# Isomorpfishm/SINGA

Measured on AMD Instinct MI355X. Metric: protein-ligand graphs/sec GAN step (G+D fwd+bwd); scatter-TP kernel HBM GB/s, higher is better.
Workload: dtype f32

## Files before the change

### __graft_entry__.py

```python
import os
import subprocess
import sys

ROOT = os.path.dirname(os.path.abspath(__file__))
if ROOT not in sys.path:
    sys.path.insert(0, ROOT)

SRC = os.path.join(ROOT, "singa_amd", "csrc", "singa_hip.hip")
LIB = os.path.join(ROOT, "singa_amd", "lib", "libsinga_hip.so")


def build() -> None:
    os.makedirs(os.path.dirname(LIB), exist_ok=True)
    deps = [SRC, os.path.join(ROOT, "singa_amd", "csrc", "so3_index.h"), os.path.join(ROOT, "include", "singa_hip.h"),
            os.path.join(ROOT, "include", "singa_hip_lab.h"), os.path.join(ROOT, "include", "singa_hip_gen.h"),
            os.path.join(ROOT, "include", "singa_hip_force.h")]
    if not os.path.exists(LIB) or any(os.path.getmtime(d) > os.path.getmtime(LIB) for d in deps):
        hipcc = os.environ.get("HIPCC", "/opt/rocm/bin/hipcc")
        cmd = [hipcc, "--offload-arch=gfx950", "-O3", "-std=c++17", "-shared", "-fPIC", "-o", LIB, SRC]
        subprocess.check_call(cmd)
    import torch
    import singa_amd
    from singa_amd import _capi
    _capi.bind(LIB)


def smoke() -> None:
    import numpy as np
    import torch

    build()
    from oracle import singa_oracle as O
    from singa_amd import graph as G
    from singa_amd.config import load_config
    from singa_amd.model.GAN import SINGA
    from tests.helpers import golden, state_from_spec

    assert torch.cuda.is_available(), "smoke() needs a GPU"
    L = 2
    dev = "cuda:0"
    sd = state_from_spec(f"singa_L{L}")
    z = golden(f"singa_L{L}_B3.npz")
    names = ["3wi2_4tpp", "4agq_5a7b", "5cp5_4nue"]
    batch = G.collate([G.load_npz(os.path.join(ROOT, "tests", "golden", f"graph_{n}.npz"), with_lap=False) for n in names])
    batch.nodes[G.PA]["lap_pe"], batch.nodes[G.LA]["lap_pe"] = torch.tensor(z["lap_p"]), torch.tensor(z["lap_l"])
    batch.extras["edge_rot_mat"] = {k: torch.tensor(z[f"rot_{k}"]) for k in ("pp", "ll", "lp")}
    batch.extras["knn"] = {G.PA: torch.tensor(z["knn_p"]), G.LA: torch.tensor(z["knn_l"])}
    batch = batch.to(dev)
    model = SINGA(load_config(lmax=L), device=dev)
    model.load_state_dict(sd, strict=False)
    model.eval()
    logits = model(batch)
    loss = torch.nn.functional.cross_entropy(logits, batch["ligand_data"]["smiIndices_tgt"].reshape(-1))
    loss.backward()
    torch.cuda.synchronize()
    og = O.collate([O.load_graph_npz(os.path.join(ROOT, "tests", "golden", f"graph_{n}.npz")) for n in names])
    rots = {k: torch.as_tensor(z[f"rot_{k}"]) for k in ("pp", "ll", "lp")}
    with torch.no_grad():
        ref = O.singa_forward(sd, og, rots, L, torch.as_tensor(z["knn_p"]), torch.as_tensor(z["knn_l"]),
                              torch.as_tensor(z["lap_p"]), torch.as_tensor(z["lap_l"]))
    err = float((logits.detach().cpu().double() - ref.double()).norm() / ref.double().norm())
    gn = float(torch.sqrt(sum((p.grad.double() ** 2).sum() for p in model.parameters() if p.grad is not None)))
    print(f"smoke: loss {float(loss):.6f} (reference {float(z['loss']):.6f}), logits rel err vs oracle {err:.2e}, "
          f"grad norm {gn:.4f} (reference {float(z['grad_total']):.4f})")
    assert err < 1e-4, err
    assert abs(gn - float(z["grad_total"])) < 1e-4 * float(z["grad_total"])


if __name__ == "__main__":
    build()
    if len(sys.argv) > 1 and sys.argv[1] == "smoke":
        smoke()
```

### singa_amd/_capi.py

```python
import ctypes as C

P = C.c_void_p
I32 = C.c_int
I64 = C.c_int64
F32 = C.c_float


class Seg(C.Structure):
    _fields_ = [("ptr", P), ("ld", I64), ("rows", C.c_int32)]


SegArr = Seg * 3


class Gemm(C.Structure):
    _fields_ = [("a", P), ("b", P), ("c", P), ("bias", P), ("lda", I64), ("ldb", I64), ("ldc", I64), ("I", C.c_int32),
                ("J", C.c_int32), ("R", C.c_int32), ("a_group", C.c_int32), ("b_group", C.c_int32), ("c_group", C.c_int32),
                ("a_group_ld", I64), ("b_group_ld", I64), ("c_group_ld", I64), ("c_split_stride", I64), ("mask", P),
                ("addend", P), ("relu", C.c_int32), ("asum", P), ("asum_stride", I64)]


class CGemm(C.Structure):
    _fields_ = [("a", P), ("b", P), ("c", P), ("lda", I64), ("ldb", I64), ("ldc", I64), ("a_im", I64), ("b_im", I64),
                ("c_im", I64), ("c_split_stride", I64), ("I", C.c_int32), ("J", C.c_int32), ("R", C.c_int32),
# ... 33 lines not shown
    "singa_s2act_sep_fwd": ([C.POINTER(Seg), I32, P, I64, P, P, P, P, I32, I32, I32, P], I32),
    "singa_s2act_sep_bwd": ([C.POINTER(Seg), I32, P, I64, P, P, P, P, P, P, I32, I32, I32, P], I32),
    "singa_s2act_ffn_bwd": ([P, P, I64, P, P, P, P, P, P, I32, I32, I32, P], I32),
    "singa_s2act_sep_bwd_seg": ([C.POINTER(Seg), I32, P, I64, P, P, P, P, C.POINTER(Seg), P, I64, I32, I32, I32, P], I32),
    "singa_so3_rmsnorm_nparts": ([I32], I32),
    "singa_so3_rmsnorm_fwd": ([P, P, P, P, I32, I32, I32, F32, P], I32),
    "singa_so3_rmsnorm_bwd": ([P, P, P, P, P, P, I32, I32, I32, F32, P], I32),
    "singa_so3_rmsnorm_bwd_add": ([P, P, P, P, P, P, P, I32, I32, I32, F32, P], I32),
    "singa_edge_logits_fwd": ([P] * 7 + [I32, I32, I32, F32, P], I32),
    "singa_edge_logits_bwd": ([P] * 13 + [I32, I32, I32, F32, P], I32),
    "singa_gather_wsum_fwd": ([P] * 6 + [I32, I32, I32, P], I32),
    "singa_gather_wsum_bwd": ([P] * 12 + [I32, I32, I32, P], I32),
    "singa_bias_ssp_fwd": ([P] * 3 + [I64, I32, P], I32),
    "singa_bias_ssp_bwd": ([P] * 4 + [I64, I32, P], I32),
    "singa_dec_self_attn": ([P] * 10 + [I32, I32, P, F32, P], I32),
    "singa_dec_cross_attn": ([P] * 10 + [I32, I32, I32, P, F32, P], I32),
    "singa_dec_ffn": ([P] * 7 + [I32, P, F32, P], I32),
    "singa_sample_token": ([P, P, P, P, I32, I32, I32, I32, F32, I32, F32, I32, I32] + [P] * 8, I32),
    "singa_edge_mlp_fwd": ([P] * 11 + [I32, I32, I32, I32, P], I32),
    "singa_edge_mlp_bwd_nparts": ([I32, I32], I32),
    "singa_edge_mlp_bwd": ([P] * 6 + [I32, I32, I32, P], I32),
    "singa_masked_softmax_fwd": ([P, P, I64, I64, P, I32, I32, I32, I32, F32, P], I32),
    "singa_masked_softmax_bwd": ([P, P, P, I64, I64, P, I32, I32, I32, I32, F32, P], I32),
    "singa_attn_fwd": ([P, P, P, P, I64, I64, P, P, I32, I32, I32, I32, I32, I32, I32, I64, I64, I64, F32, P], I32),
    "singa_attn_bwd": ([P, P, P, P, I64, I64] + [P] * 7 + [I32, I32, I32, I32, I32, I32, I32, I64, I64, I64, F32, P], I32),
    "singa_ln256_nparts": ([I64], I32),
    "singa_ln256_fwd": ([P] * 5 + [I64, I32, F32, P], I32),
    "singa_ln256_bwd": ([P] * 6 + [I64, I32, F32, P], I32),
    "singa_ln_silu_nparts": ([I64], I32),
    "singa_ln_silu_fwd": ([P] * 4 + [I64, I32, F32, P], I32),
    "singa_ln_silu_bwd": ([P] * 6 + [I64, I32, F32, P], I32),
    "singa_colsum_work": ([C.c_longlong, I32], C.c_longlong),
    "singa_colsum": ([P, C.c_longlong, C.c_longlong, I32, P, P, P], I32),
    "singa_so3_skinny_nparts": ([I32, I32, I32], I32),
    "singa_so3_skinny_expand": ([P, P, I64, I64, I64, P, P, I32, I32, I32, P], I32),
    "singa_so3_skinny_reduce": ([P, P, P, I32, I32, I32, I32, I32, P], I32),
    "singa_colsum_multi_work": ([C.c_longlong, I32], C.c_longlong),
    "singa_colsum_multi": ([I32, P, P, P, P, P, I32, P, P, P, C.c_longlong, P], I32),
    "singa_block_weight_fwd": ([P, P, I32, I32, P], I32),
    "singa_block_weight_bwd": ([P, P, I32, I32, I32, P], I32),
    "singa_rowdot_nparts": ([C.c_longlong], I32),
    "singa_rowdot_fwd": ([P, P, P, C.c_longlong, I32, F32, P], I32),
    "singa_rowdot_bwd": ([P, P, P, P, P, C.c_longlong, I32, F32, P], I32),
    "singa_lap_pe_work": ([I32, I32], I32),
    "singa_lap_pe": ([P] * 8 + [I32, I32, I32, P], I32),
    "singa_adam_step": ([P, P, P, P, P, P, P, I32, I32, P, P, F32, F32, F32, P], I32),
    "singa_grad_norm": ([P, P, P, P, I32, I32, P, P, P], I32),
    "singa_gemm_f32": ([C.POINTER(Gemm), I32, I32, I32, I32, P], I32),
    "singa_cgemm3m_f32": ([C.POINTER(CGemm), I32, I32, I32, I32, P], I32),
    "singa_knn_graph": ([P, P, P, I32, I32, I32, I32, P, P, P], I32),
    "singa_knn_edge_attr": ([P, P, C.c_longlong, P, C.c_float, P, I32, I32, P], I32),
    "singa_prof_enable": ([I32], I32),
    "singa_prof_hint_edges": ([I32], I32),
    "singa_prof_collect": ([P, P, P, I32], I32),
    "singa_prof_collect_tagged": ([P, P, P, P, I32], I32),
    "singa_prof_stamps": ([P, I32], I32),
    "singa_prof_read_stamps": ([P, P, P, P, P, I32], I32),
    "singa_prof_reset": ([], I32),
    "singa_calib_copy": ([P, P, C.c_longlong, P], I32),
    "singa_calib_copy16": ([P, P, C.c_longlong, I32, I32, P], I32),
}

EXPORTS = tuple(_SIGS)

_LAB_SIGS = {
    "singa_so3_skinny_variant": ([I32], I32),
    "singa_gemm_occupancy": ([I32, I32, I32], I32),
    "singa_gemm_force_cfg": ([I32], I32),
    "singa_lap_pe_fsi_min": ([I32], I32),
}
LAB_EXPORTS = tuple(_LAB_SIGS)

_GEN_SIGS = {
    "singa_sample_token_grammar": ([P, P, P, P, P, I32, I32, I32, I32, F32, I32, F32, I32, I32] + [P] * 10, I32),
    "singa_smiles_rule_host": ([P, P, P, I32, P, P], I32),
}
GEN_EXPORTS = tuple(_GEN_SIGS)

_FORCE_SIGS = {
    "singa_sample_token_forced": ([P, P, P, P, P, I32, I32, I32, I32, F32, I32, F32, I32, I32] + [P] * 12, I32),
}
FORCE_EXPORTS = tuple(_FORCE_SIGS)


def bind(path):
    import torch
    lib = C.CDLL(path)
    for name, (args, res) in list(_SIGS.items()) + list(_LAB_SIGS.items()) + list(_GEN_SIGS.items()) + \
            list(_FORCE_SIGS.items()):
        fn = getattr(lib, name)
        fn.argtypes = args
        fn.restype = res
    return lib


def segs(items):
    arr = SegArr()
    for i, (p, ld, rows) in enumerate(items):
        arr[i].ptr, arr[i].ld, arr[i].rows = p, ld, rows
    return arr, len(items)


def check(lib, code, what):
    if code != 0:
        raise RuntimeError(f"{what} failed ({code}): {lib.singa_last_error_string().decode()}")
```

### singa_amd/csrc/singa_hip.hip

```cpp
#include <hip/hip_runtime.h>
#include <hip/hip_ext.h>

#include <math.h>
#include <stdint.h>
#include <stdio.h>
#include <string.h>
#include <type_traits>

#include "../../include/singa_hip.h"
#include "../../include/singa_hip_lab.h"
#include "../../include/singa_hip_gen.h"
#include "../../include/singa_hip_force.h"
#include "so3_index.h"

namespace {

thread_local char g_err[256] = "ok";

int fail(int code, const char* msg) {
    snprintf(g_err, sizeof(g_err), "%s", msg);
    return code;
}

int check_launch(const char* what) {
    hipError_t e = hipGetLastError();
    if (e != hipSuccess) {
        snprintf(g_err, sizeof(g_err), "%s: %s", what, hipGetErrorString(e));
        return (int)e;
    }
    return SINGA_OK;
}

struct ProfRec {
    hipEvent_t a, b;
    int E, N, tag;
};
constexpr int PROF_CAP = 8192;
ProfRec g_prof[PROF_CAP];
int g_prof_n = 0;
bool g_prof_on = false;
unsigned long long* g_stamp_buf = nullptr;
int g_stamp_cap = 0;
__global__ void stamp_kernel(unsigned long long* dst) { *dst = (unsigned long long)wall_clock64(); }
int g_prof_edges_hint = 0;

#ifndef SINGA_KEEP_VGPR
#define SINGA_KEEP_VGPR(x) __asm__ volatile("" : "+v"(x))
#endif

#define SINGA_LAUNCH(tag_, E_, N_, kern, grid, block, st, ...)                                                   \
    do {                                                                                                          \
        if (g_prof_on && g_prof_n < PROF_CAP) {                                                                   \
            ProfRec& r_ = g_prof[g_prof_n++];                                                                     \
            (void)hipEventCreate(&r_.a);                                                                          \
            (void)hipEventCreate(&r_.b);                                                                          \
            r_.E = (E_);                                                                                          \
            r_.N = (N_);                                                                                          \
            r_.tag = (tag_);                                                                                      \
            hipExtLaunchKernelGGL(kern, grid, block, 0, (st), r_.a, r_.b, 0, __VA_ARGS__);                        \
        } else if (g_stamp_buf && 2 * (g_prof_n + 2) <= g_stamp_cap && g_prof_n + 1 < PROF_CAP) {                 \
            if (g_prof_n == 0) {                                                                                  \
                g_prof[0].a = g_prof[0].b = nullptr;                                                              \
                g_prof[0].E = g_prof[0].N = g_prof[0].tag = 0;                                                    \
                hipLaunchKernelGGL(stamp_kernel, dim3(1), dim3(1), 0, (st), g_stamp_buf);                         \
                hipLaunchKernelGGL(stamp_kernel, dim3(1), dim3(1), 0, (st), g_stamp_buf + 1);                     \
                g_prof_n = 1;                                                                                     \
            }                                                                                                     \
            ProfRec& r_ = g_prof[g_prof_n];                                                                       \
            r_.a = r_.b = nullptr;                                                                                \
            r_.E = (E_);                                                                                          \
            r_.N = (N_);                                                                                          \
            r_.tag = (tag_);                                                                                      \
            hipLaunchKernelGGL(stamp_kernel, dim3(1), dim3(1), 0, (st), g_stamp_buf + 2 * g_prof_n);              \
            hipLaunchKernelGGL(kern, grid, block, 0, (st), __VA_ARGS__);                                          \
            hipLaunchKernelGGL(stamp_kernel, dim3(1), dim3(1), 0, (st), g_stamp_buf + 2 * g_prof_n + 1);          \
            ++g_prof_n;                                                                                           \
        } else                                                                                                    \
            hipLaunchKernelGGL(kern, grid, block, 0, (st), __VA_ARGS__);                                          \
    } while (0)

__device__ __forceinline__ int xcd_range_id(int vb, int n8) { return (vb & 7) * (n8 >> 3) + (vb >> 3); }
constexpr int MAX_J = 2300;
__device__ float g_J[MAX_J];
int g_lmax_init = -1;

__host__ __device__ constexpr int j_off(int l) {
    int s = 0;
    for (int i = 0; i < l; ++i) s += (2 * i + 1) * (2 * i + 1);
    return s;
}

struct Segs {
    const float* p[3];
    long long ld[3];
    int rows[3];
// ... 3207 lines not shown
        auto load = [&](float4* b, float* a, int q, int ch) {
            const int n = q + g;
            const bool ok = n < n1;
            const long long nn = ok ? n : n1 - 1;
#pragma unroll
            for (int d = 0; d < D; ++d) {
                const int k = ch * D + d;
                b[d] = *reinterpret_cast<const float4*>(big + (nn * K + k) * C + cc);
                const float v = small[(nn * K + k) * 16 + i];
                a[d] = ok ? v : 0.f;
            }
        };
        load(bnxt, anxt, n0, 0);
        for (int q = n0; q < n1; q += 4) {
#pragma unroll
            for (int ch = 0; ch < NCH; ++ch) {
#pragma unroll
                for (int d = 0; d < D; ++d) bcur[d] = bnxt[d], acur[d] = anxt[d];
                if (ch + 1 < NCH) load(bnxt, anxt, q, ch + 1);
                else load(bnxt, anxt, q + 4 < n1 ? q + 4 : q, 0);
#pragma unroll
                for (int d = 0; d < D; ++d) {
                    const int k = ch * D + d;
                    int l = 0;
                    while ((l + 1) * (l + 1) <= k) ++l;
                    const float bv[4] = {bcur[d].x, bcur[d].y, bcur[d].z, bcur[d].w};
#pragma unroll
                    for (int t = 0; t < 4; ++t) acc[l][t] = __builtin_amdgcn_mfma_f32_16x16x4f32(acur[d], bv[t], acc[l][t], 0, 0, 0);
                    if (k == 0 && q + g < n1) {
                        accb.x += bv[0]; accb.y += bv[1]; accb.z += bv[2]; accb.w += bv[3];
                    }
                }
            }
        }
    }
    constexpr int WSZ_ = (L + 1) * 16 * C;
    float* p = part + (long long)(blockIdx.x / HV) * (WSZ_ + (bias_row ? C : 0));
    if (bias_row) {
        accb.x += __shfl_xor(accb.x, 16, 64); accb.y += __shfl_xor(accb.y, 16, 64); accb.z += __shfl_xor(accb.z, 16, 64); accb.w += __shfl_xor(accb.w, 16, 64);
        accb.x += __shfl_xor(accb.x, 32, 64); accb.y += __shfl_xor(accb.y, 32, 64); accb.z += __shfl_xor(accb.z, 32, 64); accb.w += __shfl_xor(accb.w, 32, 64);
    }
    if (!act) return;
#pragma unroll
    for (int l = 0; l <= L; ++l) {
        if (out_cu) {
#pragma unroll
            for (int t = 0; t < 4; ++t)
                *reinterpret_cast<float4*>(p + ((long long)l * C + cc + t) * 16 + 4 * g) = make_float4(acc[l][t][0], acc[l][t][1], acc[l][t][2], acc[l][t][3]);
        } else {
#pragma unroll
            for (int r = 0; r < 4; ++r)
                *reinterpret_cast<float4*>(p + ((long long)l * 16 + 4 * g + r) * C + cc) = make_float4(acc[l][0][r], acc[l][1][r], acc[l][2][r], acc[l][3][r]);
        }
    }
    if (bias_row && g == 0) *reinterpret_cast<float4*>(p + WSZ_ + cc) = accb;
}

static inline int so3_skinny_npb(int N, int target_blocks) {
    int npb = (N + target_blocks - 1) / target_blocks;
    return npb < 8 ? 8 : npb;
}

template <int C>
static int so3_skinny_reduce_runs(int lmax) {
    static int cached[8] = {0};
    if (lmax < 0 || lmax > 7) return 512;
    if (cached[lmax]) return cached[lmax];
    int per_cu = 0, cus = 256;
    hipError_t e = hipErrorInvalidValue;
    constexpr int BL = SkinnyCfg<C>::BLOCK;
    if (lmax == 2) e = hipOccupancyMaxActiveBlocksPerMultiprocessor(&per_cu, so3_skinny_reduce_kernel<2, C>, BL, 0);
    if (lmax == 4) e = hipOccupancyMaxActiveBlocksPerMultiprocessor(&per_cu, so3_skinny_reduce_kernel<4, C>, BL, 0);
    if (lmax == 6) e = hipOccupancyMaxActiveBlocksPerMultiprocessor(&per_cu, so3_skinny_reduce_kernel<6, C>, BL, 0);
    if (e != hipSuccess || per_cu < 1) per_cu = 2;
    int dev = 0;
    hipDeviceProp_t prop;
    if (hipGetDevice(&dev) == hipSuccess && hipGetDeviceProperties(&prop, dev) == hipSuccess && prop.multiProcessorCount > 0)
        cus = prop.multiProcessorCount;
    cached[lmax] = per_cu * cus / SkinnyCfg<C>::HALVES;
    return cached[lmax];
}
static inline bool so3_skinny_channels_ok(int C) { return C == 512 || C == 112; }

__device__ __forceinline__ float group16_sum(float v) {
    v += __shfl_xor(v, 1, 64);
    v += __shfl_xor(v, 2, 64);
    v += __shfl_xor(v, 4, 64);
    v += __shfl_xor(v, 8, 64);
    return v;
}
__host__ __device__ constexpr int deg_of_c(int k) {
    int l = 0;
    while ((l + 1) * (l + 1) <= k) ++l;
    return l;
}
__host__ __device__ constexpr float bal_of_c(int k, int L) { return 1.0f / (float)((2 * deg_of_c(k) + 1) * (L + 1)); }

template <int L>
__global__ void __launch_bounds__(64) rmsnorm_fwd4_kernel(const float* __restrict__ x, const float* __restrict__ weight,
                                                          const float* __restrict__ bias, float* __restrict__ y, int N, float eps) {
    constexpr int C = 16, K = (L + 1) * (L + 1), KC = K * C;
    const int lane = threadIdx.x, q = lane >> 4, c = lane & 15;
    float w[L + 1];
#pragma unroll
    for (int l = 0; l <= L; ++l) w[l] = weight[l * C + c];
    const float bc = bias[c];
    for (int n0 = 4 * (int)blockIdx.x; n0 < N; n0 += 4 * (int)gridDim.x) {
        const int n = n0 + q;
        const bool ok = n < N;
        const float* xi = x + (long long)(ok ? n : N - 1) * KC + c;
        float v[K];
#pragma clang loop unroll(full)
        for (int k = 0; k < K; ++k) v[k] = xi[k * C];
        v[0] -= group16_sum(v[0]) * (1.0f / C);
        float ss = 0.f;
#pragma clang loop unroll(full)
        for (int k = 0; k < K; ++k) ss = fmaf(v[k] * v[k], bal_of_c(k, L), ss);
        const float r = rsqrtf(group16_sum(ss) * (1.0f / C) + eps);
        if (ok) {
            float* yo = y + (long long)n * KC + c;
#pragma clang loop unroll(full)
            for (int k = 0; k < K; ++k) {
                const float rw = r * w[deg_of_c(k)];
                yo[k * C] = k == 0 ? fmaf(v[k], rw, bc) : v[k] * rw;
            }
        }
    }
}

template <int L, bool ADD>
__global__ void __launch_bounds__(64) rmsnorm_bwd4_kernel(const float* __restrict__ x, const float* __restrict__ weight,
                                                          const float* __restrict__ gy, const float* __restrict__ g_add,
                                                          float* __restrict__ gx, float* __restrict__ gw_part,
                                                          float* __restrict__ gb_part, int N, float eps) {
    constexpr int C = 16, K = (L + 1) * (L + 1), KC = K * C;
    const int lane = threadIdx.x, q = lane >> 4, c = lane & 15;
    float w[L + 1], gwp[L + 1];
#pragma unroll
    for (int l = 0; l <= L; ++l) { w[l] = weight[l * C + c]; gwp[l] = 0.f; }
    float gbp = 0.f;
    for (int n0 = 4 * (int)blockIdx.x; n0 < N; n0 += 4 * (int)gridDim.x) {
        const int n = n0 + q;
        const bool ok = n < N;
        const long long base = (long long)(ok ? n : N - 1) * KC + c;
        float v[K], g[K], ga[ADD ? K : 1];
#pragma clang loop unroll(full)
        for (int k = 0; k < K; ++k) {
            v[k] = x[base + k * C];
            g[k] = gy[base + k * C];
            if constexpr (ADD) ga[k] = g_add[base + k * C];
        }
        const float live = ok ? 1.f : 0.f;
        v[0] -= group16_sum(v[0]) * (1.0f / C);
        float ss = 0.f, gl[L + 1];
#pragma unroll
        for (int l = 0; l <= L; ++l) gl[l] = 0.f;
#pragma clang loop unroll(full)
        for (int k = 0; k < K; ++k) {
            ss = fmaf(v[k] * v[k], bal_of_c(k, L), ss);
            gl[deg_of_c(k)] = fmaf(g[k], v[k], gl[deg_of_c(k)]);
        }
        float S = 0.f;
#pragma unroll
        for (int l = 0; l <= L; ++l) S = fmaf(gl[l], w[l], S);
        gbp = fmaf(g[0], live, gbp);
        const float r = rsqrtf(group16_sum(ss) * (1.0f / C) + eps);
// ... 2150 lines not shown
        o[i].ld = kin * C;
        o[i].rows = x[i].rows;
        at += x[i].rows;
    }
    return singa_s2act_sep_bwd_seg(x, nseg, gate, ldg, P, Q, A, g_out, o, g_gate, C, E, C, lmax, stream);
}


int singa_so3_skinny_nparts(int N, int lmax, int C) {
    if (N <= 0 || !so3_skinny_channels_ok(C)) return 0;
    const int runs = C == 512 ? so3_skinny_reduce_runs<512>(lmax) : so3_skinny_reduce_runs<112>(lmax);
    const int npb = so3_skinny_npb(N, runs);
    return (N + npb - 1) / npb;
}

#define SINGA_SKINNY_LC(lmax, C, ...)                                                      \
    do {                                                                                   \
        if ((C) == 512) {                                                                  \
            constexpr int C_ = 512;                                                        \
            switch (lmax) {                                                                \
                case 2: { constexpr int L_ = 2; __VA_ARGS__; } break;                      \
                case 4: { constexpr int L_ = 4; __VA_ARGS__; } break;                      \
                case 6: { constexpr int L_ = 6; __VA_ARGS__; } break;                      \
                default: return fail(SINGA_E_LMAX, "so3_skinny: lmax must be 2, 4 or 6");  \
            }                                                                              \
        } else {                                                                           \
            constexpr int C_ = 112;                                                        \
            switch (lmax) {                                                                \
                case 2: { constexpr int L_ = 2; __VA_ARGS__; } break;                      \
                case 4: { constexpr int L_ = 4; __VA_ARGS__; } break;                      \
                case 6: { constexpr int L_ = 6; __VA_ARGS__; } break;                      \
                default: return fail(SINGA_E_LMAX, "so3_skinny: lmax must be 2, 4 or 6");  \
            }                                                                              \
        }                                                                                  \
    } while (0)

static int g_skinny_valu = 0;
int singa_so3_skinny_variant(int valu) {
    g_skinny_valu = valu ? 1 : 0;
    return SINGA_OK;
}

int singa_so3_skinny_expand(const float* small, const float* W, long long w_l, long long w_c, long long w_u, const float* bias,
                            float* big, int N, int C, int lmax, void* stream) {
    if (!small || !W || !big) return fail(SINGA_E_NULL, "so3_skinny_expand: null pointer");
    if (!so3_skinny_channels_ok(C)) return fail(SINGA_E_SHAPE, "so3_skinny: built for 512 and 112 wide channels");
    if (((uintptr_t)small & 15) || ((uintptr_t)big & 15) || (bias && ((uintptr_t)bias & 15)))
        return fail(SINGA_E_SHAPE, "so3_skinny_expand: 16-byte aligned tensors");
    if (N <= 0) return SINGA_OK;
    hipStream_t st = (hipStream_t)stream;
    if (g_skinny_valu) {
        const int npb = so3_skinny_npb(N, 1536);
        SINGA_SKINNY_LC(lmax, C, hipLaunchKernelGGL((so3_skinny_expand_kernel<L_, C_>),
                                                    dim3((unsigned)(SkinnyCfg<C_>::HALVES * ((N + npb - 1) / npb))),
                                                    dim3(SkinnyCfg<C_>::BLOCK), 0, st, small, W, w_l, w_c, w_u, bias, big, N, npb));
    } else {
        const int npb = (so3_skinny_npb(N, 2048) + 15) / 16 * 16;
        SINGA_SKINNY_LC(lmax, C, hipLaunchKernelGGL((so3_skinny_expand_mfma_kernel<L_, C_>),
                                                    dim3((unsigned)(SkinnyCfg<C_>::HALVES * ((N + npb - 1) / npb))),
                                                    dim3(SkinnyCfg<C_>::BLOCK), 0, st, small, W, w_l, w_c, w_u, bias, big, N, npb));
    }
    return check_launch("so3_skinny_expand");
}

int singa_so3_skinny_reduce(const float* small, const float* big, float* part, int N, int C, int lmax, int out_cu, int bias_row,
                            void* stream) {
    if (!small || !big || !part) return fail(SINGA_E_NULL, "so3_skinny_reduce: null pointer");
    if (!so3_skinny_channels_ok(C)) return fail(SINGA_E_SHAPE, "so3_skinny: built for 512 and 112 wide channels");
    if (N <= 0) return SINGA_OK;
    const int runs = C == 512 ? so3_skinny_reduce_runs<512>(lmax) : so3_skinny_reduce_runs<112>(lmax);
    const int npb = so3_skinny_npb(N, runs);
    hipStream_t st = (hipStream_t)stream;
    if (((uintptr_t)small & 15) || ((uintptr_t)big & 15) || ((uintptr_t)part & 15))
        return fail(SINGA_E_SHAPE, "so3_skinny_reduce: 16-byte aligned tensors");
    if (g_skinny_valu)
        SINGA_SKINNY_LC(lmax, C, hipLaunchKernelGGL((so3_skinny_reduce_kernel<L_, C_>),
                                                    dim3((unsigned)(SkinnyCfg<C_>::HALVES * ((N + npb - 1) / npb))),
                                                    dim3(SkinnyCfg<C_>::BLOCK), 0, st, small, big, part, N, npb, out_cu, bias_row));
    else
        SINGA_SKINNY_LC(lmax, C, hipLaunchKernelGGL((so3_skinny_reduce_mfma_kernel<L_, C_>),
                                                    dim3((unsigned)(SkinnyCfg<C_>::HALVES * ((N + npb - 1) / npb))),
                                                    dim3(SkinnyCfg<C_>::BLOCK), 0, st, small, big, part, N, npb, out_cu, bias_row));
    return check_launch("so3_skinny_reduce");
}

int singa_block_weight_fwd(const float* w, float* out, int h, int k, void* stream) {
    if (!w || !out) return fail(SINGA_E_NULL, "block_weight_fwd: null pointer");
    if (h <= 0 || k <= 0) return SINGA_OK;
    const long long n = 4LL * h * k;
    hipLaunchKernelGGL(block_weight_fwd_kernel, dim3((unsigned)((n + 255) / 256)), dim3(256), 0, (hipStream_t)stream, w, out, h, k);
    return check_launch("block_weight_fwd");
}

int singa_block_weight_bwd(const float* g_block, float* g_w, int h, int k, int accumulate, void* stream) {
    if (!g_block || !g_w) return fail(SINGA_E_NULL, "block_weight_bwd: null pointer");
    if (h <= 0 || k <= 0) return SINGA_OK;
    const long long n = 2LL * h * k;
    hipLaunchKernelGGL(block_weight_bwd_kernel, dim3((unsigned)((n + 255) / 256)), dim3(256), 0, (hipStream_t)stream, g_block, g_w, h, k,
                       accumulate);
    return check_launch("block_weight_bwd");
}

int singa_rowdot_nparts(long long M) { return M <= 0 ? 0 : (int)((M + ROWDOT_ROWS - 1) / ROWDOT_ROWS); }

int singa_rowdot_fwd(const float* x, const float* b, float* out, long long M, int D, float scale, void* stream) {
    if (!x || !b || !out) return fail(SINGA_E_NULL, "rowdot_fwd: null pointer");
    if (D != 32) return fail(SINGA_E_SHAPE, "rowdot: built for 32 channels per row");
    if (((uintptr_t)x & 15) || ((uintptr_t)b & 15)) return fail(SINGA_E_SHAPE, "rowdot: 16-byte aligned operands");
    if (M <= 0) return SINGA_OK;
    hipLaunchKernelGGL(rowdot32_fwd_kernel, dim3((unsigned)((M * 8 + 255) / 256)), dim3(256), 0, (hipStream_t)stream, x, b, out, M, scale);
    return check_launch("rowdot_fwd");
}

int singa_rowdot_bwd(const float* g, const float* x, const float* b, float* gx, float* part, long long M, int D, float scale,
                     void* stream) {
    if (!g || !x || !b || !gx || !part) return fail(SINGA_E_NULL, "rowdot_bwd: null pointer");
    if (D != 32) return fail(SINGA_E_SHAPE, "rowdot: built for 32 channels per row");
    if (((uintptr_t)x & 15) || ((uintptr_t)b & 15) || ((uintptr_t)gx & 15)) return fail(SINGA_E_SHAPE, "rowdot: 16-byte aligned operands");
    if (M <= 0) return SINGA_OK;
    hipLaunchKernelGGL(rowdot32_bwd_kernel, dim3((unsigned)singa_rowdot_nparts(M)), dim3(256), 0, (hipStream_t)stream, g, x, b, gx, part, M,
                       scale);
    return check_launch("rowdot_bwd");
}

static int g_lap_fsi_min = 384;
int singa_lap_pe_fsi_min(int n) {
    if (n < 0) return fail(SINGA_E_SHAPE, "lap_pe_fsi_min: >= 0 (a value above 896 switches the sparse route off)");
    g_lap_fsi_min = n;
    return SINGA_OK;
}

int singa_lap_pe_work(int B, int ld) {
#ifdef SINGA_EMUL
    return (B < 0 || ld < 0) ? 0 : B * (3 + 4 * 9) * ld;
#else
    return (B < 0 || ld < 0) ? 0 : B * LAP_WORK_PER_LD * ld;
#endif
}

int singa_lap_pe(double* A, const int32_t* esrc, const int32_t* edst, const int32_t* eptr, const int32_t* nnodes, const int32_t* first,
                 double* work, float* out, int B, int ld, int kout, void* stream) {
    if (!A || !esrc || !edst || !eptr || !nnodes || !first || !work || !out) return fail(SINGA_E_NULL, "lap_pe: null pointer");
    if (kout < 1 || kout > 8) return fail(SINGA_E_SHAPE, "lap_pe: 1..8 eigenvectors");
    if (ld < 1 || ld > 896) return fail(SINGA_E_SHAPE, "lap_pe: graphs of up to 896 atoms (22.5 vectors of LDS per graph)");
    if (B <= 0) return SINGA_OK;
#ifdef SINGA_EMUL
    return fail(SINGA_E_SHAPE, "lap_pe: not part of the emulation build");
#else
    const int sl = ld < 32 ? 32 : ld;
    const size_t lds = (size_t)((4 + 16) * sl + 16 + 8) * sizeof(double) + (size_t)(5 * sl + 4) * sizeof(int);
    hipStream_t st = (hipStream_t)stream;
    hipError_t e;
    if (ld <= 512) {
        e = hipFuncSetAttribute(reinterpret_cast<const void*>(lap_pe_kernel<8>), hipFuncAttributeMaxDynamicSharedMemorySize, (int)lds);
        if (e != hipSuccess) return fail((int)e, "lap_pe: LDS size refused");
        hipLaunchKernelGGL(lap_pe_kernel<8>, dim3(B), dim3(1024), lds, st, A, esrc, edst, eptr, nnodes, first, work, out, ld, kout, g_lap_fsi_min);
    } else {
        e = hipFuncSetAttribute(reinterpret_cast<const void*>(lap_pe_kernel<16>), hipFuncAttributeMaxDynamicSharedMemorySize, (int)lds);
        if (e != hipSuccess) return fail((int)e, "lap_pe: LDS size refused");
        hipLaunchKernelGGL(lap_pe_kernel<16>, dim3(B), dim3(1024), lds, st, A, esrc, edst, eptr, nnodes, first, work, out, ld, kout, g_lap_fsi_min);
    }
    return check_launch("lap_pe");
#endif
}

int singa_adam_step(float* const* p, const float* const* g, float* const* m, float* const* v, const long long* sizes,
// ... 668 lines not shown
```

### singa_amd/ops.py

```python
import ctypes
import math
import warnings

import torch

warnings.filterwarnings("ignore", message=".*preferred_blas_library is an experimental feature.*")

from . import _capi, _lib, so3


PROFILE_ON = False


def profile_start(in_graph=False):
    global PROFILE_ON, _STAMPS
    PROFILE_ON = True
    if in_graph:
        _STAMPS = torch.zeros(2 * 8192 + 2, dtype=torch.int64, device="cuda")
        _chk(_lib.lib().singa_prof_stamps(_p(_STAMPS), _STAMPS.numel()), "singa_prof_stamps")
    else:
        _chk(_lib.lib().singa_prof_enable(1), "singa_prof_enable")


_STAMPS = None
# ... 1056 lines not shown
            q = total = 0
            for k, (src, segs) in enumerate(jobs):
                xs[k], lds[k], Ms[k], ns_[k], seg0[k] = src.data_ptr(), src.stride(0), src.shape[0], src.shape[1], q
                total += lib.singa_colsum_multi_work(src.shape[0], src.shape[1])
                for c0, g in segs:
                    col0[q], dst[q] = c0, g.data_ptr()
                    q += 1
            work = torch.empty(max(total, 1), device=jobs[0][0].device, dtype=torch.float32)
            _chk(lib.singa_colsum_multi(nj, xs, lds, Ms, ns_, seg0, ns, col0, dst, _p(work), total, _stream()),
                 "singa_colsum_multi")


def param_colsum(src, targets):
    src = src.reshape(src.shape[0], math.prod(src.shape[1:]))
    if src.stride(1) != 1:
        src = src.contiguous()
    direct = [src.shape[0] > 0 and _GradSink.takes(t[2]) for t in targets]
    out = [None] * len(targets)
    i = 0
    while i < len(targets):
        j = i
        while j + 1 < len(targets) and direct[j + 1] == direct[i]:
            j += 1
        c0, c1 = targets[i][0], targets[j][0] + targets[j][1]
        blk = src[:, c0:c1]
        if direct[i]:
            _GradSink.jobs.append((blk, [(t[0] - c0, t[2].grad) for t in targets[i:j + 1]]))
        else:
            tot = colsum(blk)
            for k in range(i, j + 1):
                out[k] = tot[targets[k][0] - c0: targets[k][0] - c0 + targets[k][1]]
        i = j + 1
    return out


class _BiasAdd(torch.autograd.Function):
    @staticmethod
    def forward(ctx, x, b):
        ctx.param = b
        return x + b

    @staticmethod
    def backward(ctx, g):
        n = g.shape[-1]
        return g, param_colsum(g.reshape(-1, n), [(0, n, ctx.param)])[0]


def bias_add(x, b):
    return _BiasAdd.apply(x, b)


class _rocblas:

    def __enter__(self):
        torch.backends.cuda.preferred_blas_library("cublas")

    def __exit__(self, *a):
        torch.backends.cuda.preferred_blas_library("cublaslt")
        return False


class _BmmSmall(torch.autograd.Function):

    @staticmethod
    def forward(ctx, a, b):
        ctx.save_for_backward(a, b)
        with _rocblas():
            return torch.bmm(a, b)

    @staticmethod
    def backward(ctx, g):
        a, b = ctx.saved_tensors
        with _rocblas():
            ga = torch.bmm(g, b.transpose(1, 2)) if ctx.needs_input_grad[0] else None
            gb = torch.bmm(a.transpose(1, 2), g) if ctx.needs_input_grad[1] else None
        return ga, gb


def bmm_small(a, b):
    return _BmmSmall.apply(a, b)


USE_SKINNY_SO3 = True
_GEMM_SPLIT_ROWS = 2048


def _rows(t):
    if t.stride(-1) != 1 or t.stride(0) % 4 or t.data_ptr() % 16:
        t = t.contiguous()
    return t


def _mat(t, what):
    if t.dim() == 2:
        (rows, cols), ld, grp, gld = t.shape, t.stride(0), 0, 0
    elif t.dim() == 3:
        (n, grp, cols), gld, ld = t.shape, t.stride(0), t.stride(1)
        rows = n * grp
    else:
        raise RuntimeError(f"GEMM operand {what}: a 2-D or 3-D view, got {tuple(t.shape)}")
    ptr = t.data_ptr()
    bad = ("the columns are not contiguous" if t.stride(-1) != 1 else "the base is not 16-byte aligned" if ptr % 16 else
           "the pitches are not multiples of 4 floats" if ld % 4 or gld % 4 else None)
    if bad:
        raise RuntimeError(f"GEMM operand {what}, shape {tuple(t.shape)}, strides {t.stride()}, address {ptr:#x}: {bad}")
    return ptr, rows, cols, ld, grp, gld


def _like_c(t, C, what):
    pitches = all(st == sc for st, sc, n in zip(t.stride(), C.stride(), C.shape) if n > 1)
    if t.shape != C.shape or not pitches or t.data_ptr() % 16:
        raise RuntimeError(f"GEMM {what}: shape {tuple(t.shape)}, strides {t.stride()} must be those of the result "
                         f"({tuple(C.shape)}, {C.stride()}), 16-byte aligned")
    return t.data_ptr()


def _extents(a_rc, b_rc, a, b, c, unit=""):
    (I, Ra), (J, Rb) = (a if a_rc else a[::-1]), (b if b_rc else b[::-1])
    if Ra != Rb or c != (I, J):
        raise RuntimeError(f"GEMM form ({int(a_rc)}, {int(b_rc)}): A {a}, B {b} and C {c} (rows, columns{unit}) disagree on I, J, R")
    return I, J, Ra


def _prob(A, B, C, a_rc, b_rc, bias=None, addend=None, mask=None, relu=False, asum=None):
    a, ar, ac, lda, ag, agl = _mat(A, "A")
    b, br, bc, ldb, bg, bgl = _mat(B, "B")
    c, cr, cc, ldc, cg, cgl = _mat(C, "C")
    slabs = C.dim() == 3 and not a_rc
    I, J, R = _extents(a_rc, b_rc, (ar, ac), (br, bc), (cg, cc) if slabs else (cr, cc))
    it = dict(a=a, lda=lda, b=b, ldb=ldb, c=c, ldc=ldc, I=I, J=J, R=R)
    if ag:
        it.update(a_group=ag, a_group_ld=agl)
    if bg:
        it.update(b_group=bg, b_group_ld=bgl)
    if slabs:
        if ldc != J or cgl < I * J:
            raise RuntimeError(f"GEMM slabs {tuple(C.shape)}, strides {C.stride()}: dense [I, J] blocks that do not overlap")
        it.update(c_split_stride=cgl)
    elif cg:
        it.update(c_group=cg, c_group_ld=cgl)
    if bias is not None:
        if bias.shape != (J,) or bias.stride(0) != 1 or bias.data_ptr() % 16:
            raise RuntimeError(f"GEMM bias: a contiguous 16-byte aligned [{J}], got {tuple(bias.shape)}")
        it.update(bias=bias.data_ptr())
    if addend is not None:
        it.update(addend=_like_c(addend, C, "addend"))
    if mask is not None:
        it.update(mask=_like_c(mask, C, "mask"))
    if relu:
        it.update(relu=1)
    if asum is not None:
        if (a_rc or ag or asum.dim() != 2 or asum.shape[1] != I or asum.stride(1) != 1
                or (slabs and asum.shape[0] != C.shape[0])):
            raise RuntimeError(f"GEMM asum {tuple(asum.shape)}: one contiguous row of I = {I} floats per split, (0, 0) form, plain A rows")
        it.update(asum=asum.data_ptr(), asum_stride=asum.stride(0))
    return it


def _cprob(A, B, C, a_rc, b_rc, sigma):
    parts = []
    for (re, im), what in zip((A, B, C), "ABC"):
        ptr, rows, cols, ld, grp, gld = _mat(re, what)
        off = im.data_ptr() - ptr
        if im.shape != re.shape or im.stride() != re.stride() or off % 16:
            raise RuntimeError(f"complex GEMM operand {what}: the imaginary part {tuple(im.shape)}, strides {im.stride()} must be "
                             f"laid out like the real part {tuple(re.shape)}, {re.stride()}, a multiple of 4 floats away")
# ... 126 lines not shown


class _SO2Conv3M(torch.autograd.Function):

    @staticmethod
    def forward(ctx, X, w0, b0, w1, w2, n0, n1):
        ctx.params = (w0, w1, w2, b0)
        X = _rows(X)
        ws = [_rows(w0), w1.contiguous(), w2.contiguous()]
        b0 = b0.contiguous()
        _dev(X, *ws, b0)
        E, nin = X.shape
        ins = (n0, n1, nin - n0 - n1)
        outs = tuple(w.shape[0] for w in ws)
        assert ws[0].shape[1] == n0 and all(2 * w.shape[1] == k and w.shape[0] % 2 == 0 for w, k in zip(ws[1:], ins[1:]))
        H = torch.empty(E, sum(outs), device=X.device, dtype=torch.float32)
        xs, hs = X.split(ins, 1), H.split(outs, 1)
        if E > 0:
            _gemm([_prob(xs[0], ws[0], hs[0], True, True, bias=b0)], True, True)
            _cgemm([_cprob(x.chunk(2, 1), w.chunk(2, 0), h.chunk(2, 1), True, True, 1.0)
                    for x, w, h in zip(xs[1:], ws[1:], hs[1:])], True, True)
        ctx.save_for_backward(X, *ws)
        ctx.ins = ins
        return hs

    @staticmethod
    def backward(ctx, g0, g1, g2):
        X, *ws = ctx.saved_tensors
        ins, outs = ctx.ins, tuple(w.shape[0] for w in ws)
        E = X.shape[0]
        gs = [_rows(g) for g in (g0, g1, g2)]
        xs = X.split(ins, 1)
        S0 = _splits_few(E, -(-outs[0] // 128) * -(-ins[0] // 128))
        Sc = _splits_few(E, sum(-(-(o // 2) // 128) * -(-(k // 2) // 64) for o, k in zip(outs[1:], ins[1:])))
        pw0, pw1, pw2, pb0 = ctx.params
        (gw0,), (gb,) = _dw_grads([(gs[0], xs[0], pw0, pb0)], S0)
        (gw1, gw2), _ = _dw_grads([(gs[1], xs[1], pw1, None), (gs[2], xs[2], pw2, None)], Sc, cplx=True)
        gX = None
        if ctx.needs_input_grad[0]:
            gX = torch.empty_like(X)
            if E > 0:
                gxs = gX.split(ins, 1)
                _gemm([_prob(gs[0], ws[0], gxs[0], True, False)], True, False)
                _cgemm([_cprob(g.chunk(2, 1), w.chunk(2, 0), gx.chunk(2, 1), True, False, -1.0)
                        for g, w, gx in zip(gs[1:], ws[1:], gxs[1:])], True, False)
        return gX, gw0, gb, gw1, gw2, None, None


def so2_conv3m(X, w0, b0, w1, w2, n0, n1):
    return _SO2Conv3M.apply(X, w0, b0, w1, w2, n0, n1)


def so2_linear3(X, w0, b0, w1, w2, n0, n1):
    return _SO2Linear3.apply(X, w0, b0, w1, w2, n0, n1)


def _degrees(t, L):
    return t.split([2 * l + 1 for l in range(L + 1)], 1)


def _so3_linear_probs(x, weight, out, L, b_rc, bias=None, addend=None):
    if weight.shape[0] != L + 1:
        raise RuntimeError(f"SO3 linear: {weight.shape[0]} weight matrices for the degrees 0..{L}")
    ads = _degrees(addend, L) if addend is not None else [None] * (L + 1)
    return [_prob(a, w, c, True, b_rc, bias=bias if l == 0 else None, addend=ad)
            for l, (a, w, c, ad) in enumerate(zip(_degrees(x, L), weight.unbind(0), _degrees(out, L), ads))]


class _SO3Linear(torch.autograd.Function):

    @staticmethod
    def forward(ctx, x, weight, bias, L, addend=None):
        ctx.params = (weight, bias)
        x, weight, bias = x.contiguous(), weight.contiguous(), bias.contiguous()
        _dev(x, weight, bias)
        N, K, cin = x.shape
        cout = weight.shape[1]
        out = torch.empty(N, K, cout, device=x.device, dtype=torch.float32)
        ctx.has_addend = addend is not None
        if addend is not None:
            addend = addend.contiguous()
            _dev(addend)
            assert addend.shape == out.shape and not (USE_SKINNY_SO3 and cin == 16 and cout == 512)
        if USE_SKINNY_SO3 and cin == 16 and cout == 512:
            _chk(_lib.lib().singa_so3_skinny_expand(_p(x), _p(weight), cout * cin, cin, 1, _p(bias), _p(out), N, cout, L,
                                                    _stream()), "singa_so3_skinny_expand")
        elif N > 0:
            _gemm(_so3_linear_probs(x, weight, out, L, True, bias, addend), True, True)
        ctx.save_for_backward(x, weight)
        ctx.L = L
        return out

    @staticmethod
    def backward(ctx, g):
        x, weight = ctx.saved_tensors
        L = ctx.L
        g = g.contiguous()
        N, K, cin = x.shape
        cout = weight.shape[1]
        lib = _lib.lib()
        skinny = USE_SKINNY_SO3 and N > 0 and ((cin == 16 and cout == 512) or (cin in (512, 112) and cout == 16))
        wide = max(cin, cout)
        gx = None
        if ctx.needs_input_grad[0]:
            gx = torch.empty_like(x)
            if skinny and cout == 16:
                _chk(lib.singa_so3_skinny_expand(_p(g), _p(weight), cout * cin, 1, cin, None, _p(gx), N, wide, L, _stream()),
                     "singa_so3_skinny_expand(dx)")
            elif N > 0:
                _gemm(_so3_linear_probs(g, weight, gx, L, False), True, False)
        if skinny:
            wide_out = cout == wide
            wsz = (L + 1) * 16 * wide
            part = torch.empty(lib.singa_so3_skinny_nparts(N, L, wide), wsz + (wide if wide_out else 0), device=x.device,
                               dtype=torch.float32)
            small, big = (x, g) if wide_out else (g, x)
            _chk(lib.singa_so3_skinny_reduce(_p(small), _p(big), _p(part), N, wide, L, int(wide_out), int(wide_out), _stream()),
                 "singa_so3_skinny_reduce")
            if wide_out:
                gw, gb = param_colsum(part, [(0, wsz, ctx.params[0]), (wsz, wide, ctx.params[1])])
            else:
                gw = param_colsum(part, [(0, wsz, ctx.params[0])])[0]
                gb = param_colsum(g[:, 0, :], [(0, cout, ctx.params[1])])[0]
            return gx, (gw.view(L + 1, cout, cin) if gw is not None else None), gb, None, (g if ctx.has_addend else None)
        (gw,), _ = _dw_grads([(gl, xl, ctx.params[0], None) for gl, xl in zip(_degrees(g, L), _degrees(x, L))],
                             _splits_for(N * (2 * L + 1)))
        return gx, gw, param_colsum(g[:, 0, :], [(0, cout, ctx.params[1])])[0], None, (g if ctx.has_addend else None)


def so3_linear(x, weight, bias, L, addend=None):
    return _SO3Linear.apply(x, weight, bias, L, addend)


class _FFNTail(torch.autograd.Function):

    @staticmethod
    def forward(ctx, h, gate, weight, bias, L, addend=None):
        ctx.params = (weight, bias)
        h, gate, weight, bias = h.contiguous(), gate.contiguous(), weight.contiguous(), bias.contiguous()
        _dev(h, gate, weight, bias)
        N, K, cin = h.shape
        cout = weight.shape[1]
        assert cin == 512 and cout == 16 and weight.shape[2] == cin
        lib = _lib.lib()
        P, Q, A = _grid_factors(L, L, False, h.device)
        a = torch.empty_like(h)
        seg, n = _capi.segs([(h.data_ptr(), K * cin, K)])
        _chk(lib.singa_s2act_sep_fwd(seg, n, _p(gate), gate.stride(0), _p(P), _p(Q), _p(A), _p(a), N, cin, L, _stream()),
             "singa_s2act_sep_fwd(node)")
        out = torch.empty(N, K, cout, device=h.device, dtype=torch.float32)
        ctx.has_addend = addend is not None
        if addend is not None:
            addend = addend.contiguous()
            _dev(addend)
            assert addend.shape == out.shape
        if N > 0:
            _gemm(_so3_linear_probs(a, weight, out, L, True, bias, addend), True, True)
        ctx.save_for_backward(h, gate, a, weight)
        ctx.L = L
        return out

    @staticmethod
    def backward(ctx, g):
        h, gate, a, weight = ctx.saved_tensors
        L = ctx.L
        g = g.contiguous()
        N, K, cin = h.shape
        cout = weight.shape[1]
        lib = _lib.lib()
        P, Q, _ = _grid_factors(L, L, False, h.device)
        gh, gg = torch.empty_like(h), torch.empty_like(gate)
        if N > 0:
            _chk(lib.singa_s2act_ffn_bwd(_p(h), _p(gate), gate.stride(0), _p(P), _p(Q), _p(g), _p(weight), _p(gh), _p(gg), N, cin, L,
                                         _stream()), "singa_s2act_ffn_bwd")
        wsz = (L + 1) * 16 * cin
        gw = None
        if N > 0:
            part = torch.empty(lib.singa_so3_skinny_nparts(N, L, cin), wsz, device=h.device, dtype=torch.float32)
            _chk(lib.singa_so3_skinny_reduce(_p(g), _p(a), _p(part), N, cin, L, 0, 0, _stream()), "singa_so3_skinny_reduce")
            gw = param_colsum(part, [(0, wsz, ctx.params[0])])[0]
        else:
            gw = torch.zeros(wsz, device=h.device, dtype=torch.float32)
        gb = param_colsum(g[:, 0, :], [(0, cout, ctx.params[1])])[0]
        return gh, gg, (gw.view(L + 1, cout, cin) if gw is not None else None), gb, None, (g if ctx.has_addend else None)


# ... 377 lines not shown
```

Measured before the change: 861.7.

## Fuse skinny SO3 linear backward dx and dW/db into one MFMA pass

Adds a matrix-core kernel for the 16->512 SO3 linear backward that reads the wide gradient once. In a single pass it computes the input gradient (g·W) and the per-block partial weight and bias sums. Previously two separate kernels each streamed the large gradient tensor. The new kernel carries complex wave-level LDS staging and a heavy register footprint, and its occupancy is sized at runtime.

```diff
diff --git a/__graft_entry__.py b/__graft_entry__.py
--- a/__graft_entry__.py
+++ b/__graft_entry__.py
@@ -14,7 +14,7 @@
     os.makedirs(os.path.dirname(LIB), exist_ok=True)
     deps = [SRC, os.path.join(ROOT, "singa_amd", "csrc", "so3_index.h"), os.path.join(ROOT, "include", "singa_hip.h"),
             os.path.join(ROOT, "include", "singa_hip_lab.h"), os.path.join(ROOT, "include", "singa_hip_gen.h"),
-            os.path.join(ROOT, "include", "singa_hip_force.h")]
+            os.path.join(ROOT, "include", "singa_hip_force.h"), os.path.join(ROOT, "include", "singa_hip_ffn.h")]
     if not os.path.exists(LIB) or any(os.path.getmtime(d) > os.path.getmtime(LIB) for d in deps):
         hipcc = os.environ.get("HIPCC", "/opt/rocm/bin/hipcc")
         cmd = [hipcc, "--offload-arch=gfx950", "-O3", "-std=c++17", "-shared", "-fPIC", "-o", LIB, SRC]
diff --git a/include/singa_hip_ffn.h b/include/singa_hip_ffn.h
--- /dev/null
+++ b/include/singa_hip_ffn.h
@@ -0,0 +1,12 @@
+#ifndef SINGA_HIP_FFN_H
+#define SINGA_HIP_FFN_H
+#ifdef __cplusplus
+extern "C" {
+#endif
+int singa_so3_skinny_pair_nparts(int N, int lmax, int C);
+int singa_so3_skinny_bwd_pair(const float* small, const float* big, const float* W, float* g_small, float* part, int N, int C,
+                              int lmax, void* stream);
+#ifdef __cplusplus
+}
+#endif
+#endif
diff --git a/singa_amd/_capi.py b/singa_amd/_capi.py
--- a/singa_amd/_capi.py
+++ b/singa_amd/_capi.py
@@ -139,12 +139,18 @@
 }
 FORCE_EXPORTS = tuple(_FORCE_SIGS)
 
+_FFN_SIGS = {
+    "singa_so3_skinny_pair_nparts": ([I32, I32, I32], I32),
+    "singa_so3_skinny_bwd_pair": ([P, P, P, P, P, I32, I32, I32, P], I32),
+}
+FFN_EXPORTS = tuple(_FFN_SIGS)
+
 
 def bind(path):
     import torch
     lib = C.CDLL(path)
     for name, (args, res) in list(_SIGS.items()) + list(_LAB_SIGS.items()) + list(_GEN_SIGS.items()) + \
-            list(_FORCE_SIGS.items()):
+            list(_FORCE_SIGS.items()) + list(_FFN_SIGS.items()):
         fn = getattr(lib, name)
         fn.argtypes = args
         fn.restype = res
diff --git a/singa_amd/csrc/singa_hip.hip b/singa_amd/csrc/singa_hip.hip
--- a/singa_amd/csrc/singa_hip.hip
+++ b/singa_amd/csrc/singa_hip.hip
@@ -11,6 +11,7 @@
 #include "../../include/singa_hip_lab.h"
 #include "../../include/singa_hip_gen.h"
 #include "../../include/singa_hip_force.h"
+#include "../../include/singa_hip_ffn.h"
 #include "so3_index.h"
 
 namespace {
@@ -3384,6 +3385,172 @@
 }
 static inline bool so3_skinny_channels_ok(int C) { return C == 512 || C == 112; }
 
+#ifndef SINGA_EMUL
+template <int V>
+struct SkinnyInt { static constexpr int value = V; };
+template <int B, int E, class F>
+__device__ __forceinline__ void skinny_steps(F&& f) {
+    if constexpr (B < E) {
+        f(SkinnyInt<B>{});
+        skinny_steps<B + 1, E>(f);
+    }
+}
+constexpr int skinny_degree(int k) {
+    int l = 0;
+    while ((l + 1) * (l + 1) <= k) ++l;
+    return l;
+}
+__device__ __forceinline__ void skinny_wave_sync() {
+    __builtin_amdgcn_fence(__ATOMIC_RELEASE, "wavefront");
+    __builtin_amdgcn_wave_barrier();
+    __builtin_amdgcn_fence(__ATOMIC_ACQUIRE, "wavefront");
+}
+template <int L, int C>
+__global__ void __launch_bounds__(C) __attribute__((amdgpu_waves_per_eu(2, 2))) so3_skinny_bwd_pair_mfma_kernel(const float* __restrict__ small, const float* __restrict__ big,
+                                                                     const float* __restrict__ W, float* __restrict__ g_small,
+                                                                     float* __restrict__ part, int N, int npb) {
+    constexpr int K = (L + 1) * (L + 1), D = SkinnyChunk<L>::D, NCH = K / D, NW = C / 64;
+    static_assert(NCH * D == K && C == 512, "chunking / one workgroup = 8 slabs");
+    __shared__ floatx4 img[NW][256];
+    __shared__ float4 px[2][NW][D * 64];
+    const int wave = threadIdx.x >> 6, lane = threadIdx.x & 63, i = lane & 15, g = lane >> 4;
+    const int cw = wave * 64;
+    const int cc = cw + 4 * i;
+    const int n0 = (int)blockIdx.x * npb;
+    const int n1 = n0 + npb < N ? n0 + npb : N;
+    if (n0 >= n1) return;
+    floatx4 acc[L + 1][4];
+#pragma unroll
+    for (int l = 0; l <= L; ++l)
+#pragma unroll
+        for (int t = 0; t < 4; ++t) acc[l][t] = floatx4{0.f, 0.f, 0.f, 0.f};
+    float4 accb = make_float4(0.f, 0.f, 0.f, 0.f);
+    floatx4 bcur[4], bnxt[4];
+    float acur[4], anxt[4];
+    const float* brun = big + (long long)n0 * K * C;
+    const float* srun = small + (long long)n0 * K * 16;
+    unsigned bo[4], so[4];
+    auto tile_rows = [&](int nb) {
+#pragma unroll
+        for (int qd = 0; qd < 4; ++qd) {
+            const int n = nb + 4 * qd + g;
+            const unsigned r = (unsigned)((n < n1 ? n : n1 - 1) - n0) * K;
+            bo[qd] = r * C + cc;
+            so[qd] = r * 16 + i;
+        }
+    };
+    auto load = [&](floatx4* b, float* a, int k) {
+#pragma unroll
+        for (int qd = 0; qd < 4; ++qd) {
+            b[qd] = *reinterpret_cast<const floatx4*>(brun + (bo[qd] + (unsigned)(k * C)));
+            a[qd] = srun[so[qd] + (unsigned)(k * 16)];
+        }
+    };
+    float wx[4][4];
+    tile_rows(n0);
+    load(bnxt, anxt, 0);
+    float* pxf = reinterpret_cast<float*>(&px[0][0][0]);
+    int pb = 0;
+    for (int nb = n0; nb < n1; nb += 16) {
+        int wo = cw + 4 * g;
+        asm volatile("" : "+v"(wo));
+        skinny_steps<0, K>([&](auto kc) {
+            constexpr int k = decltype(kc)::value, ch = k / D, d = k - ch * D, l = skinny_degree(k);
+#pragma unroll
+            for (int qd = 0; qd < 4; ++qd) bcur[qd] = bnxt[qd], acur[qd] = anxt[qd];
+            if (k == l * l) {
+#pragma unroll
+                for (int m = 0; m < 4; ++m)
+#pragma unroll
+                    for (int j = 0; j < 4; ++j) wx[m][j] = W[(l * C + wo + 16 * m + j) * 16 + i];
+            }
+            if (k + 1 < K) load(bnxt, anxt, k + 1);
+            else {
+                tile_rows(nb + 16 < n1 ? nb + 16 : nb);
+                load(bnxt, anxt, 0);
+            }
+            __builtin_amdgcn_sched_barrier(0);
+#pragma unroll
+            for (int qd = 0; qd < 4; ++qd) asm volatile("" : "+v"(bcur[qd]), "+v"(acur[qd]));
+#pragma unroll
+            for (int qd = 0; qd < 4; ++qd) {
+                const float bv[4] = {bcur[qd][0], bcur[qd][1], bcur[qd][2], bcur[qd][3]};
+                const bool ok = nb + 4 * qd + g < n1;
+                const float a = ok ? acur[qd] : 0.f;
+#pragma unroll
+                for (int t = 0; t < 4; ++t) acc[l][t] = __builtin_amdgcn_mfma_f32_16x16x4f32(a, bv[t], acc[l][t], 0, 0, 0);
+                if (k == 0 && ok) {
+                    accb.x += bv[0]; accb.y += bv[1]; accb.z += bv[2]; accb.w += bv[3];
+                }
+            }
+#pragma unroll
+            for (int qd = 0; qd < 4; ++qd) {
+                const int row = 4 * qd + g;
+                img[wave][row * 16 + (i ^ row)] = bcur[qd];
+            }
+            skinny_wave_sync();
+            floatx4 ax = floatx4{0.f, 0.f, 0.f, 0.f};
+#pragma unroll
+            for (int m = 0; m < 4; ++m) {
+                const floatx4 v = img[wave][i * 16 + ((g + 4 * m) ^ i)];
+                const float av[4] = {v[0], v[1], v[2], v[3]};
+#pragma unroll
+                for (int j = 0; j < 4; ++j) ax = __builtin_amdgcn_mfma_f32_16x16x4f32(av[j], wx[m][j], ax, 0, 0, 0);
+            }
+            skinny_wave_sync();
+            float* o = pxf + (pb * NW + wave) * (D * 256);
+#pragma unroll
+            for (int r = 0; r < 4; ++r) o[((4 * g + r) * D + d) * 16 + i] = ax[r];
+            if (d == D - 1) {
+                __syncthreads();
+                if ((int)threadIdx.x < D * 64) {
+                    const int e = 4 * (int)threadIdx.x, node = e / (D * 16), rem = e - node * (D * 16);
+                    float4 s = px[pb][0][threadIdx.x];
+#pragma unroll
+                    for (int w = 1; w < NW; ++w) {
+                        const float4 v = px[pb][w][threadIdx.x];
+                        s.x += v.x; s.y += v.y; s.z += v.z; s.w += v.w;
+                    }
+                    if (nb + node < n1)
+                        *reinterpret_cast<float4*>(g_small + ((long long)(nb + node) * K + ch * D) * 16 + rem) = s;
+                }
+                pb ^= 1;
+            }
+        });
+    }
+    constexpr int WSZ_ = (L + 1) * 16 * C;
+    float* p = part + (long long)blockIdx.x * (WSZ_ + C);
+    accb.x += __shfl_xor(accb.x, 16, 64); accb.y += __shfl_xor(accb.y, 16, 64); accb.z += __shfl_xor(accb.z, 16, 64); accb.w += __shfl_xor(accb.w, 16, 64);
+    accb.x += __shfl_xor(accb.x, 32, 64); accb.y += __shfl_xor(accb.y, 32, 64); accb.z += __shfl_xor(accb.z, 32, 64); accb.w += __shfl_xor(accb.w, 32, 64);
+#pragma unroll
+    for (int l = 0; l <= L; ++l)
+#pragma unroll
+        for (int t = 0; t < 4; ++t)
+            *reinterpret_cast<float4*>(p + ((long long)l * C + cc + t) * 16 + 4 * g) = make_float4(acc[l][t][0], acc[l][t][1], acc[l][t][2], acc[l][t][3]);
+    if (g == 0) *reinterpret_cast<float4*>(p + WSZ_ + cc) = accb;
+}
+
+static int so3_skinny_pair_npb(int N, int lmax) {
+    static int cached[8] = {0};
+    int runs = 256;
+    if (lmax >= 0 && lmax <= 7 && cached[lmax]) runs = cached[lmax];
+    else if (lmax == 2 || lmax == 4 || lmax == 6) {
+        int per_cu = 0, cus = 256;
+        hipError_t e = hipErrorInvalidValue;
+        if (lmax == 2) e = hipOccupancyMaxActiveBlocksPerMultiprocessor(&per_cu, so3_skinny_bwd_pair_mfma_kernel<2, 512>, 512, 0);
+        if (lmax == 4) e = hipOccupancyMaxActiveBlocksPerMultiprocessor(&per_cu, so3_skinny_bwd_pair_mfma_kernel<4, 512>, 512, 0);
+        if (lmax == 6) e = hipOccupancyMaxActiveBlocksPerMultiprocessor(&per_cu, so3_skinny_bwd_pair_mfma_kernel<6, 512>, 512, 0);
+        if (e != hipSuccess || per_cu < 1) per_cu = 1;
+        int dev = 0;
+        hipDeviceProp_t prop;
+        if (hipGetDevice(&dev) == hipSuccess && hipGetDeviceProperties(&prop, dev) == hipSuccess && prop.multiProcessorCount > 0)
+            cus = prop.multiProcessorCount;
+        runs = cached[lmax] = per_cu * cus;
+    }
+    return (so3_skinny_npb(N, runs) + 15) / 16 * 16;
+}
+#endif
+
 __device__ __forceinline__ float group16_sum(float v) {
     v += __shfl_xor(v, 1, 64);
     v += __shfl_xor(v, 2, 64);
@@ -5700,6 +5867,40 @@
                                                     dim3((unsigned)(SkinnyCfg<C_>::HALVES * ((N + npb - 1) / npb))),
                                                     dim3(SkinnyCfg<C_>::BLOCK), 0, st, small, big, part, N, npb, out_cu, bias_row));
     return check_launch("so3_skinny_reduce");
+}
+
+int singa_so3_skinny_pair_nparts(int N, int lmax, int C) {
+    if (N <= 0 || C != 512 || (lmax != 2 && lmax != 4 && lmax != 6) || g_skinny_valu) return 0;
+#ifdef SINGA_EMUL
+    return 0;
+#else
+    const int npb = so3_skinny_pair_npb(N, lmax);
+    return (N + npb - 1) / npb;
+#endif
+}
+
+int singa_so3_skinny_bwd_pair(const float* small, const float* big, const float* W, float* g_small, float* part, int N, int C,
+                              int lmax, void* stream) {
+    if (!small || !big || !W || !g_small || !part) return fail(SINGA_E_NULL, "so3_skinny_bwd_pair: null pointer");
+    if (C != 512) return fail(SINGA_E_SHAPE, "so3_skinny_bwd_pair: built for 512 wide channels");
+    if (lmax != 2 && lmax != 4 && lmax != 6) return fail(SINGA_E_LMAX, "so3_skinny_bwd_pair: lmax must be 2, 4 or 6");
+    if (((uintptr_t)small & 15) || ((uintptr_t)big & 15) || ((uintptr_t)W & 15) || ((uintptr_t)g_small & 15) || ((uintptr_t)part & 15))
+        return fail(SINGA_E_SHAPE, "so3_skinny_bwd_pair: 16-byte aligned tensors");
+    if (N <= 0) return SINGA_OK;
+    if (g_skinny_valu) return fail(SINGA_E_SHAPE, "so3_skinny_bwd_pair: a matrix-core kernel, there is no VALU variant of it");
+#ifdef SINGA_EMUL
+    return fail(SINGA_E_SHAPE, "so3_skinny_bwd_pair: not part of the emulation build");
+#else
+    const int npb = so3_skinny_pair_npb(N, lmax);
+    if ((long long)npb * (lmax + 1) * (lmax + 1) * C * 4 > 0x7fffffffLL)
+        return fail(SINGA_E_SHAPE, "so3_skinny_bwd_pair: a run of nodes spans more than 2^31 bytes");
+    const dim3 grid((unsigned)((N + npb - 1) / npb)), block(512);
+    hipStream_t st = (hipStream_t)stream;
+    if (lmax == 2) hipLaunchKernelGGL((so3_skinny_bwd_pair_mfma_kernel<2, 512>), grid, block, 0, st, small, big, W, g_small, part, N, npb);
+    if (lmax == 4) hipLaunchKernelGGL((so3_skinny_bwd_pair_mfma_kernel<4, 512>), grid, block, 0, st, small, big, W, g_small, part, N, npb);
+    if (lmax == 6) hipLaunchKernelGGL((so3_skinny_bwd_pair_mfma_kernel<6, 512>), grid, block, 0, st, small, big, W, g_small, part, N, npb);
+    return check_launch("so3_skinny_bwd_pair");
+#endif
 }
 
 int singa_block_weight_fwd(const float* w, float* out, int h, int k, void* stream) {
diff --git a/singa_amd/ops.py b/singa_amd/ops.py
--- a/singa_amd/ops.py
+++ b/singa_amd/ops.py
@@ -1162,6 +1162,7 @@
 
 
 USE_SKINNY_SO3 = True
+USE_SKINNY_PAIR = True
 _GEMM_SPLIT_ROWS = 2048
 
 
@@ -1454,7 +1455,7 @@
             addend = addend.contiguous()
             _dev(addend)
             assert addend.shape == out.shape and not (USE_SKINNY_SO3 and cin == 16 and cout == 512)
-        if USE_SKINNY_SO3 and cin == 16 and cout == 512:
+        if USE_SKINNY_SO3 and cin == 16 and cout == 512 and N > 0:
             _chk(_lib.lib().singa_so3_skinny_expand(_p(x), _p(weight), cout * cin, cin, 1, _p(bias), _p(out), N, cout, L,
                                                     _stream()), "singa_so3_skinny_expand")
         elif N > 0:
@@ -1474,6 +1475,17 @@
         skinny = USE_SKINNY_SO3 and N > 0 and ((cin == 16 and cout == 512) or (cin in (512, 112) and cout == 16))
         wide = max(cin, cout)
         gx = None
+        nparts = 0
+        if skinny and USE_SKINNY_PAIR and cin == 16 and cout == 512 and ctx.needs_input_grad[0] and ctx.needs_input_grad[1]:
+            nparts = lib.singa_so3_skinny_pair_nparts(N, L, cout)
+        if nparts > 0:
+            wsz = (L + 1) * 16 * cout
+            gx = torch.empty_like(x)
+            part = torch.empty(nparts, wsz + cout, device=x.device, dtype=torch.float32)
+            _chk(lib.singa_so3_skinny_bwd_pair(_p(x), _p(g), _p(weight), _p(gx), _p(part), N, cout, L, _stream()),
+                 "singa_so3_skinny_bwd_pair")
+            gw, gb = param_colsum(part, [(0, wsz, ctx.params[0]), (wsz, cout, ctx.params[1])])
+            return gx, (gw.view(L + 1, cout, cin) if gw is not None else None), gb, None, (g if ctx.has_addend else None)
         if ctx.needs_input_grad[0]:
             gx = torch.empty_like(x)
             if skinny and cout == 16:
```

Result: no change. 859.9 (-0.2%).
